# tberriel/OVO

Measured on AMD Instinct MI355X. Metric: frames/s (CLIP+SAM2+fusion+query), 640x480 ScanNet, 1/2/4/8 MI355X, higher is better.
Workload: dtype bf16; 1 GPU; BASELINE.json configs[2]: PE-Core-L14-336 TextRegion descriptors (2 x 336^2 crops of a 640x480 frame) + SAM2 hiera_b+ image encoder @1024^2 + back-projection + cull/project/match/vote on a 1000000-point map + multi-view fusion + dense per-point fusion + 10-prompt instance and dense-map query; every frame a keyframe; masks from the precomputed-mask seam (32/frame); map_points=1000000, texts=10, masks_per_frame=32, sam2=image encoder, masks=precomputed-mask seam (mask_generator.py:94-95), encoder_batch=14, dense_query=resident class map, rows touched by the keyframe re-evaluated, parallelism=single GPU, points_end=1366868, instances_end=242

## Files before the change

### include/ovo_hip.h

```cpp
#ifndef OVO_HIP_H
#define OVO_HIP_H

#include <stddef.h>
#include <stdint.h>

#ifdef __cplusplus
extern "C" {
#endif

#define OVO_OK 0
#define OVO_E_ARG (-1)
#define OVO_E_LAUNCH (-2)
#define OVO_E_UNSUPPORTED (-3)

typedef void *ovo_stream_t;

const char *ovo_hip_last_error(void);
int ovo_hip_abi_version(void);

int ovo_marker(int id, ovo_stream_t stream);
int ovo_profile_start(void);
int ovo_profile_stop(double *ms, double *work, int64_t *launches, int n_kinds);
int ovo_profile_bytes(double *bytes, int n_kinds);

// ... 80 lines not shown


typedef struct {
    const void *A; int64_t lda;
    const void *W; int64_t ldw;
    const float *bias;
    void *C; int64_t ldc;
    const float *add; int64_t ld_add;
    int32_t M, N, K;
    int32_t in_dtype, out_dtype, act;
    float alpha;
} ovo_gemm_t;
int ovo_gemm(const ovo_gemm_t *g, ovo_stream_t stream);
typedef struct {
    const float *cos, *sin;
    int32_t T, hd, cols, t0;
} ovo_rope_t;
int ovo_gemm_rope(const ovo_gemm_t *g, const ovo_rope_t *rope, ovo_stream_t stream);
int ovo_gemm_periodic(const ovo_gemm_t *g, int64_t add_rows, ovo_stream_t stream);
typedef struct {
    int32_t B, H, W, wh, ww;
} ovo_window_t;
int ovo_gemm_unwindow(const ovo_gemm_t *g, const ovo_window_t *win, ovo_stream_t stream);
int ovo_gemm_rowln(const ovo_gemm_t *g, const ovo_window_t *win, const float *ln_g, const float *ln_b, float eps, void *ln_out, int64_t ld_ln,
                   ovo_stream_t stream);
int ovo_gemm_fold_out(const ovo_gemm_t *g, void *xb, int64_t ld_xb, float *stats, int64_t ld_stats, ovo_stream_t stream);
int ovo_gemm_fold_stats(const float *x, int64_t ldx, int M, int D, void *xb, int64_t ld_xb, float *stats, ovo_stream_t stream);
int ovo_gemm_fold_in(const ovo_gemm_t *g, const ovo_rope_t *rope, const float *stats, int64_t ld_stats, int parts, int D, const float *rowsum, float eps,
                     ovo_stream_t stream);
int ovo_gemm_f32a(const ovo_gemm_t *g, const ovo_window_t *win, const float *x, int d, const float *gamma, const float *beta,
                  float eps, int mode, int pool2x2, ovo_stream_t stream);
int ovo_mlp_f32(float *x, int64_t rows, int d, const float *ln_g, const float *ln_b, float eps, const void *w1, int64_t ldw1,
                const float *b1, int hidden, const void *w2, int64_t ldw2, const float *b2, ovo_stream_t stream);
int ovo_window_attention_f32(const float *x, int B, int H, int W, int window, int d, int d_out, int heads, int pool, const float *ln_g,
                             const float *ln_b, float eps, const void *qkv_w, int64_t ldw, const float *qkv_b, void *att, int ld_att,
                             ovo_stream_t stream);
int ovo_gemm_argmax(const ovo_gemm_t *g, uint64_t *best, int store_scores, int n_valid, ovo_stream_t stream);
int ovo_decode_best(const uint64_t *best, int64_t n, float th, int64_t *out_cls, float *out_conf, ovo_stream_t stream);

typedef struct {
    const void *q, *k, *v;
    void *o;
    int64_t q_sb, q_sh, q_st, k_sb, k_sh, k_st, v_sb, v_sh, v_st, o_sb, o_sh, o_st;
    int32_t B, H, Tq, Tk, hd;
    float scale;
    int32_t causal;
} ovo_attention_t;
int ovo_attention(const ovo_attention_t *a, ovo_stream_t stream);

int ovo_gemm_fewrows(const ovo_gemm_t *g, ovo_stream_t stream);
int ovo_attention_short(const void *qkv, int B, int T, int H, int hd, float scale, void *out, ovo_stream_t stream);
int ovo_merge_clips(const float *logits, int64_t ld_logits, int per_row, const float *clips, int B, int D, float *out, ovo_stream_t stream);

int ovo_layernorm(const float *x, int64_t x_stride, int64_t rows, int d, const float *gamma, const float *beta,
                  float eps, void *y, int64_t y_stride, int out_dtype, ovo_stream_t stream);

int ovo_vit_embed(const float *patch, const float *prefix, int n_prefix, const float *pos, int B, int P, int d,
                  const float *gamma, const float *beta, float eps, float *x, ovo_stream_t stream);

int ovo_im2col(const float *img, int B, int C, int H, int W, int ksz, int stride, int pad, void *out, int kpad,
               ovo_stream_t stream);

int ovo_resize_normalize(const void *src, int src_dtype, int C, int H, int W, int y0, int x0, int ch, int cw,
                         float *out, int oh, int ow, int antialias, float scale, const float *mean3_host,
                         const float *std3_host, ovo_stream_t stream);

// ... 225 lines not shown
```

### ovo_amd/_lib.py

```python
from __future__ import annotations

import ctypes as C
import os
from typing import Optional

import torch

_HERE = os.path.dirname(os.path.abspath(__file__))
SO_PATH = os.path.join(_HERE, "lib", "libovo_hip.so")
ABI_VERSION = 15
E_UNSUPPORTED = -3


class OvoHipError(RuntimeError):
    pass


class Camera(C.Structure):
    _fields_ = [("aabb", C.c_float * 6), ("planes", C.c_float * 24), ("w2c", C.c_float * 16),
                ("K", C.c_float * 9), ("th", C.c_float), ("h", C.c_int32), ("w", C.c_int32)]


class Ratio(C.Structure):
    _fields_ = [("enabled", C.c_int32), ("r_h", C.c_float), ("r_w", C.c_float), ("crop_edge", C.c_int32)]


_P, _I64, _I32, _F32, _SZ = C.c_void_p, C.c_int64, C.c_int, C.c_float, C.c_size_t
_CAM = C.POINTER(Camera)


class Gemm(C.Structure):
    _fields_ = [("A", _P), ("lda", _I64), ("W", _P), ("ldw", _I64), ("bias", _P), ("C", _P), ("ldc", _I64),
                ("add", _P), ("ld_add", _I64), ("M", C.c_int32), ("N", C.c_int32), ("K", C.c_int32),
                ("in_dtype", C.c_int32), ("out_dtype", C.c_int32), ("act", C.c_int32), ("alpha", _F32)]


class Rope(C.Structure):
    _fields_ = [("cos", _P), ("sin", _P), ("T", C.c_int32), ("hd", C.c_int32), ("cols", C.c_int32), ("t0", C.c_int32)]


class Window(C.Structure):
    _fields_ = [(n, C.c_int32) for n in ("B", "H", "W", "wh", "ww")]

# ... 109 lines not shown
    "ovo_mask_or": (_I32, [_P, _I64, _P, _I32, _P]),
    "ovo_gather_rows": (_I32, [_P, _I64, _P, _I32, _P, _P]),
    "ovo_mask_area": (_I32, [_P, _I64, _P, _I32, _P, _P]),
    "ovo_gemm": (_I32, [C.POINTER(Gemm), _P]),
    "ovo_gemm_argmax": (_I32, [C.POINTER(Gemm), _P, _I32, _I32, _P]),
    "ovo_gemm_rope": (_I32, [C.POINTER(Gemm), C.POINTER(Rope), _P]),
    "ovo_gemm_periodic": (_I32, [C.POINTER(Gemm), _I64, _P]),
    "ovo_gemm_unwindow": (_I32, [C.POINTER(Gemm), C.POINTER(Window), _P]),
    "ovo_gemm_fold_out": (_I32, [C.POINTER(Gemm), _P, _I64, _P, _I64, _P]),
    "ovo_gemm_fold_stats": (_I32, [_P, _I64, _I32, _I32, _P, _I64, _P, _P]),
    "ovo_gemm_fold_in": (_I32, [C.POINTER(Gemm), C.POINTER(Rope), _P, _I64, _I32, _I32, _P, _F32, _P]),
    "ovo_gemm_rowln": (_I32, [C.POINTER(Gemm), C.POINTER(Window), _P, _P, _F32, _P, _I64, _P]),
    "ovo_gemm_f32a": (_I32, [C.POINTER(Gemm), C.POINTER(Window), _P, C.c_int, _P, _P, C.c_float, C.c_int, C.c_int, _P]),
    "ovo_decode_best": (_I32, [_P, _I64, _F32, _P, _P, _P]),
    "ovo_attention": (_I32, [C.POINTER(Attention), _P]),
    "ovo_gemm_fewrows": (_I32, [C.POINTER(Gemm), _P]),
    "ovo_attention_short": (_I32, [_P, _I32, _I32, _I32, _I32, _F32, _P, _P]),
    "ovo_merge_clips": (_I32, [_P, _I64, _I32, _P, _I32, _I32, _P, _P]),
    "ovo_layernorm": (_I32, [_P, _I64, _I64, _I32, _P, _P, _F32, _P, _I64, _I32, _P]),
    "ovo_vit_embed": (_I32, [_P, _P, _I32, _P, _I32, _I32, _I32, _P, _P, _F32, _P, _P]),
    "ovo_im2col": (_I32, [_P, _I32, _I32, _I32, _I32, _I32, _I32, _I32, _P, _I32, _P]),
    "ovo_resize_normalize": (_I32, [_P, _I32, _I32, _I32, _I32, _I32, _I32, _I32, _I32, _P, _I32, _I32, _I32, _F32,
                                    C.POINTER(C.c_float), C.POINTER(C.c_float), _P]),
    "ovo_resize_normalize_batch": (_I32, [_P, _I32, _I32, _I32, _I32, _I32, _P, _I32, _P, _I32, _I32, _I32, _F32, _P, _P, _P]),
    "ovo_resize_window_normalize": (_I32, [_P, _I32, _I32, _I32, _I32, _I32, _I32, _I32, _I32, _P, _I32, _I32, _I32, _I32, _I32, _I32, _I32, _F32,
                                           C.POINTER(C.c_float), C.POINTER(C.c_float), _P]),
    "ovo_rope_qk": (_I32, [_P, _I32, _I32, _I32, _I32, _P, _P, _I32, _P]),
    "ovo_feature_masks": (_I32, [_P, _I32, _I32, _I32, _I32, _I32, _P, _I32, _P, _P]),
    "ovo_stitch_tokens_t": (_I32, [_P, _I32, _I32, _I32, _I32, _I32, _I32, _P, _I32, _P]),
    "ovo_unit_tokens": (_I32, [_P, _I32, _I32, _I32, _P, _P, _P]),
    "ovo_global_patch_filter": (_I32, [_P, _P, _I32, _I32, _I32, _F32, _P, _P]),
    "ovo_scale_rows_bf16": (_I32, [_P, _P, _I32, _I32, _P, _P]),
    "ovo_mlp_f32": (_I32, [_P, _I64, _I32, _P, _P, _F32, _P, _I64, _P, _I32, _P, _I64, _P, _P]),
    "ovo_window_attention_f32": (_I32, [_P, _I32, _I32, _I32, _I32, _I32, _I32, _I32, _I32, _P, _P, _F32, _P, _I64, _P, _P, _I32, _P]),
    "ovo_l2_normalize_rows": (_I32, [_P, _I64, _I32, _P, _P]),
    "ovo_cast_f32": (_I32, [_P, _I64, _P, _I32, _P]),
    "ovo_row_epilogue": (_I32, [_P, _I64, _I32, _P, _I64, _P, _P, _F32, _P, _I64, _P, _P, _P, _P]),
    "ovo_sam_upscale_ln": (_I32, [_P, _P, _P, _P, _P, _F32, _I64, _I32, _I32, _P, _P]),
    "ovo_sam_upscale_masks": (_I32, [_P, _P, _P, _P, _I32, _I32, _I64, _I32, _I32, _P, _P]),
    "ovo_sam_linear": (_I32, [_P, _P, _P, _P, _I64, _I32, _P, _I32, _I64, _I32, _I32, _P]),
    "ovo_sam_proj_ln": (_I32, [_P, _P, _P, _P, _P, _I64, _P, _P, _F32, _P, _I64, _P, _P, _P, _I64, _I32, _I32, _P]),
    "ovo_sam_up1_ln": (_I32, [_P, _P, _P, _P, _P, _P, _F32, _I64, _I32, _I32, _I32, _P, _P]),
    "ovo_sam_up2_masks": (_I32, [_P, _P, _P, _P, _P, _I32, _I32, _I64, _I32, _I32, _I32, _P, _P]),
    "ovo_instance_moments": (_I32, [_P, _P, _I64, _I32, _P, _P, _P]),
    "ovo_near_fraction": (_I32, [_P, _P, _P, _I32, _I64, _F32, _P, _P]),
    "ovo_remap_instances": (_I32, [_P, _I64, _P, _I32, _P]),
    "ovo_map_reanchor_workspace_bytes": (_SZ, [_I32]),
    "ovo_map_reanchor": (_I32, [_P, _P, _P, _P, _I64, _P, _P, _P, _P, _I64, _P, _P, _P, _I32, _P, _SZ, _P]),
    "ovo_sam_i2t_attention": (_I32, [_P, _I64, _I32, _P, _P, _P, _I64, _I32, _I32, _I32, _F32, _P]),
    "ovo_sam_t2i_attention": (_I32, [_P, _P, _P, _I64, _I32, _P, _I64, _I32, _I32, _I32, _F32, _P]),
    "ovo_paint_segmap": (_I32, [_P, _I32, _I64, _P, _P]),
    "ovo_amg_mask_stats": (_I32, [_P, _I32, _I32, _I32, _I32, _I32, _F32, _F32, _P, _P]),
    "ovo_amg_binarize": (_I32, [_P, _P, _I32, _I32, _I32, _I32, _I32, _F32, _P, _P]),
    "ovo_vit_workspace_bytes": (_SZ, [C.POINTER(VitConfig), _I32]),
    "ovo_vit_forward": (_I32, [C.POINTER(VitConfig), C.POINTER(VitWeights), _P, _I32, _P, _P, _SZ, _P]),
    "ovo_hiera_workspace_bytes": (_SZ, [C.POINTER(HieraConfig), _I32]),
    "ovo_hiera_forward": (_I32, [C.POINTER(HieraConfig), C.POINTER(HieraWeights), _P, _I32, _P, _P, _P, _P, _SZ, _P]),
    "ovo_hiera_patch_embed": (_I32, [_P, _I32, _I32, _I32, _P, _I32, _P, _P, _P, _P]),
    "ovo_eval_cell_keys": (_I32, [_P, _I64, C.POINTER(EvalGrid), _P, _P]),
    "ovo_eval_grid_records": (_I32, [_P, _P, _I64, _P, _P]),
    "ovo_knn5_labels": (_I32, [_P, _P, _I64, C.POINTER(EvalGrid), _P, _P, _I64, _P, _P, _P, _P, _P, _P]),
    "ovo_confusion": (_I32, [_P, _P, _I64, _I32, C.POINTER(C.c_int64), _I32, _P, _P, _P]),
}

_lib: Optional[C.CDLL] = None

# ... 173 lines not shown
```

### ovo_amd/build.py

```python
from __future__ import annotations

import concurrent.futures as cf
import os
import shutil
import subprocess
import sys

HERE = os.path.dirname(os.path.abspath(__file__))
CSRC = os.path.join(HERE, "csrc")
OUT_DIR = os.path.join(HERE, "lib")
OBJ_DIR = os.path.join(OUT_DIR, "obj")
SO = os.path.join(OUT_DIR, "libovo_hip.so")
ARCH = "gfx950"

COMMON = ["--offload-arch=" + ARCH, "-O3", "-std=c++17", "-fPIC", "-Wall", "-Wno-unused-function",
          "-Wno-unused-result", "-I" + os.path.join(os.path.dirname(HERE), "include")]
EXTRA = {"geometry.hip": ["-ffp-contract=off"], "evalknn.hip": ["-ffp-contract=off"], "mlp_stream.hip": ["-fno-slp-vectorize"], "gemm_stream.hip": ["-fno-slp-vectorize"],
         "winattn.hip": ["-fno-slp-vectorize"], "gemm8p.hip": ["-fno-slp-vectorize"],
         "merger.hip": ["-fno-slp-vectorize"]}


def hipcc() -> str:
    for c in (os.environ.get("HIPCC"), shutil.which("hipcc"), "/opt/rocm/bin/hipcc"):
        if c and os.path.exists(c):
            return c
    raise RuntimeError("hipcc not found: libovo_hip.so cannot be built")


def sources():
    return sorted(f for f in os.listdir(CSRC) if f.endswith(".hip"))


def _stale(target: str, deps) -> bool:
    if not os.path.exists(target):
        return True
    t = os.path.getmtime(target)
    return any(os.path.getmtime(d) > t for d in deps)


def _run(cmd, what: str) -> None:
    r = subprocess.run(cmd, capture_output=True, text=True)
    if r.returncode != 0:
        raise RuntimeError(f"{what} failed:\n{r.stdout}\n{r.stderr}")
    if r.stderr.strip():
        sys.stderr.write(r.stderr)


def _compile(src: str, flags, force: bool) -> bool:
    obj = os.path.join(OBJ_DIR, src.replace(".hip", ".o"))
    deps = [os.path.join(CSRC, src)] + [os.path.join(CSRC, h) for h in os.listdir(CSRC) if h.endswith(".h")]
    deps.append(os.path.join(os.path.dirname(HERE), "include", "ovo_hip.h"))
# ... 36 lines not shown
```

### ovo_amd/csrc/core.hip

```cpp
#include <stdarg.h>
#include <stdio.h>
#include <stdlib.h>

#include <string.h>

#include <atomic>
#include <chrono>
#include <vector>

#include "common.h"

static thread_local char g_err[512] = "";

void ovo_set_error(const char *fmt, ...) {
    va_list ap;
    va_start(ap, fmt);
    vsnprintf(g_err, sizeof(g_err), fmt, ap);
    va_end(ap);
}

namespace {
struct Rec { hipEvent_t a, b; int kind; double work, bytes; int shape[3], flags; int cslot; double per_item, fixed; };
struct Prof {
    bool on = false;
// ... 40 lines not shown
    if (!g_prof.on || g_prof.recs.empty() || !device_count) return;
    if (!g_prof.counts && hipHostMalloc((void **)&g_prof.counts, SLOTS * sizeof(int32_t), hipHostMallocDefault) != hipSuccess) { g_prof.counts = nullptr; return; }
    if (g_prof.n_counts >= SLOTS) return;
    Rec &r = g_prof.recs.back();
    r.cslot = g_prof.n_counts++; r.per_item = per_item; r.fixed = fixed;
    (void)hipMemcpyAsync(g_prof.counts + r.cslot, device_count, sizeof(int32_t), hipMemcpyDeviceToHost, s);
}

template <typename T>
static int host_wait(const T *flag, T value, int64_t timeout_us) {
    OVO_REQUIRE(flag, "null flag");
    const volatile T *f = flag;
    const auto t0 = std::chrono::steady_clock::now();
    for (unsigned spin = 0;; ++spin) {
        if (*f == value) { std::atomic_thread_fence(std::memory_order_acquire); return OVO_OK; }
        if ((spin & 255) == 255 &&
            std::chrono::duration_cast<std::chrono::microseconds>(std::chrono::steady_clock::now() - t0).count() > timeout_us) {
            ovo_set_error("ovo_host_wait: timed out after %lld us (flag %lld, expected %lld)", (long long)timeout_us, (long long)*f, (long long)value);
            return OVO_E_LAUNCH;
        }
        __builtin_ia32_pause();
    }
}

__global__ void k_marker(int id, int *sink) { if (sink && id < 0) *sink = id; }

extern "C" {
int ovo_marker(int id, ovo_stream_t stream) {
    k_marker<<<1, 1, 0, (hipStream_t)stream>>>(id, nullptr);
    OVO_CHECK_LAUNCH();
    return OVO_OK;
}
const char *ovo_hip_last_error(void) { return g_err; }
int ovo_hip_abi_version(void) { return 15; }

int ovo_profile_start(void) {
    g_prof.recs.clear();
    g_prof.used = 0;
    g_prof.n_counts = 0;
    g_prof.on = true;
    return OVO_OK;
}

int ovo_profile_stop(double *ms, double *work, int64_t *launches, int n_kinds) {
    g_prof.on = false;
    OVO_REQUIRE(ms && work && launches && n_kinds > 0 && n_kinds <= OVO_PROF_KINDS, "bad argument");
    for (int i = 0; i < n_kinds; ++i) { ms[i] = 0; work[i] = 0; launches[i] = 0; }
    for (int i = 0; i < OVO_PROF_KINDS; ++i) g_last_bytes[i] = 0;
    OVO_HIP(hipDeviceSynchronize());
    FILE *dump = getenv("OVO_PROF_DUMP") ? fopen(getenv("OVO_PROF_DUMP"), "a") : nullptr;
    for (const Rec &r : g_prof.recs) {
        float t = 0.f;
        if (hipEventElapsedTime(&t, r.a, r.b) != hipSuccess || r.kind >= n_kinds) continue;
        double wk = r.work, by = r.bytes;
        if (r.cslot >= 0 && g_prof.counts) wk = by = r.per_item * (double)g_prof.counts[r.cslot] + r.fixed;
        ms[r.kind] += t; work[r.kind] += wk; launches[r.kind] += 1; g_last_bytes[r.kind] += by;
        if (dump) fprintf(dump, "%d %d %d %d %.0f %.4f %d\n", r.kind, r.shape[0], r.shape[1], r.shape[2], wk, t, r.flags);
    }
    if (dump) fclose(dump);
    g_prof.recs.clear();
    g_prof.used = 0;
    return OVO_OK;
}

int ovo_profile_bytes(double *bytes, int n_kinds) {
    OVO_REQUIRE(bytes && n_kinds > 0 && n_kinds <= OVO_PROF_KINDS, "bad argument");
    for (int i = 0; i < n_kinds; ++i) bytes[i] = g_last_bytes[i];
// ... 18 lines not shown
```

### ovo_amd/csrc/gemm_common.h

```cpp
#pragma once
#include <hip/hip_bf16.h>
#include <hip/hip_fp16.h>

#include "common.h"

namespace ovo_gemm_detail {

typedef __attribute__((ext_vector_type(8))) __bf16 bf16x8;
typedef __attribute__((ext_vector_type(8))) _Float16 f16x8;
typedef __attribute__((ext_vector_type(4))) float f32x4;

struct GemmArgs {
    const char *A; long long lda;
    const char *W; long long ldw;
    const float *bias;
    void *C; long long ldc;
    const float *add; long long ld_add;
    int M, N, K;
    int out_dtype, act;
    float alpha;
    int nbn;
    int chunk, tiles;
    int add_rows;
    int strip;
// ... 205 lines not shown
}

inline double gemm_algorithmic_bytes(const GemmArgs &g) {
    const double mn = (double)g.M * g.N, a_bytes = g.ln_mode ? (double)g.M * g.ln_d * 4.0 : (double)g.M * g.K * 2.0;
    return a_bytes + (double)g.N * g.K * 2.0 + mn * (g.out_dtype == 0 ? 4.0 : 2.0) + (g.add ? (g.add_rows > 0 ? (double)g.add_rows * g.N * 4.0 : mn * 4.0) : 0.0) +
           (g.bias ? g.N * 4.0 : 0.0) +
           (g.xb_out ? mn * 2.0 + (double)g.M * (g.N / 64) * 8.0 : 0.0) +
           (g.fold_stats ? (double)g.M * g.fold_parts * 8.0 + g.N * 4.0 : 0.0);
}

inline bool knob_gemm_no_chunk() { return ovo_knob_set("OVO_GEMM_NO_CHUNK"); }
inline bool knob_gemm_no_stream() { return ovo_knob_set("OVO_GEMM_NO_STREAM"); }
inline OvoKnobStr knob_gemm_tile() { return ovo_knob_str("OVO_GEMM_TILE"); }
inline bool knob_gelu_poly() { return ovo_knob_set("OVO_GELU_POLY"); }
inline bool knob_8p_no_slab16() { return ovo_knob_set("OVO_8P_NO_SLAB16"); }

int gemm8p_launch(const GemmArgs &g, int bn, int in_dtype, hipStream_t s);

struct FoldOut { void *xb; long long ld_xb; float *stats; long long ld_stats; };
struct FoldIn { const float *stats; long long ld_stats; int parts; int D; const float *colsum; float eps; };
int gemm_fold_parts(int N);
bool gemm_fold_ok(int M, int N, int K);
int gemm_fold_producer(const ovo_gemm_t *p, const FoldOut &o, ovo_stream_t stream);
int gemm_fold_consumer(const ovo_gemm_t *p, const ovo_rope_t *rope, const FoldIn &f, ovo_stream_t stream);
int gemm_fold_rowstats(const float *x, long long ldx, int M, int D, void *xb, long long ld_xb, float *stats, ovo_stream_t stream);
int gemm8q_launch(const GemmArgs &g, int in_dtype, hipStream_t s);
int gemm_stream_launch(const GemmArgs &g, int in_dtype, hipStream_t s);
int gemm_f32a_stream(const ovo_gemm_t *p, const ovo_window_t *win, const float *x, int d, const float *gamma, const float *beta, float eps, int mode,
                     int pool2x2, ovo_stream_t stream, uint16_t *qpool_out = nullptr, int qpool_cols = 0);

int mlp_stream_launch(float *x, long long rows, int d, const float *ln_g, const float *ln_b, float eps, const void *w1, long long ldw1, const float *b1,
                      int hid, const void *w2, long long ldw2, const float *b2, hipStream_t s);

int gemm_unwindow_rowln(const ovo_gemm_t *p, const ovo_window_t *win, const float *ln_g, const float *ln_b, float eps, void *ln_out, long long ld_ln,
                        ovo_stream_t stream);

int win_attn_launch(const float *x, int B, int H, int W, int ws, int d, int d_out, int heads, int pool, const float *ln_g, const float *ln_b, float eps,
                    const void *qkv_w, long long ldw, const float *qkv_b, void *att, int ld_att, hipStream_t s);

}
```

### ovo_amd/csrc/hiera.hip

```cpp
#include "gemm_common.h"

namespace {

__device__ __forceinline__ uint16_t f2bf(float x) {
    const __bf16 h = (__bf16)x;
    return *(const uint16_t *)&h;
}
__device__ __forceinline__ float bf2f(uint16_t v) { return __uint_as_float((uint32_t)v << 16); }

struct Grid {
    int B, H, W, ws;
    int nwh, nww, wh, ww;
    long long rows;
};
__host__ __device__ inline Grid make_grid(int B, int H, int W, int ws) {
    Grid g; g.B = B; g.H = H; g.W = W; g.ws = ws;
    if (ws > 0) { g.wh = g.ww = ws; g.nwh = (H + ws - 1) / ws; g.nww = (W + ws - 1) / ws; }
    else { g.wh = H; g.ww = W; g.nwh = g.nww = 1; }
    g.rows = (long long)B * g.nwh * g.nww * g.wh * g.ww;
    return g;
}
__device__ __forceinline__ long long row_of(const Grid &g, int b, int y, int x) {
    const int wy = y / g.wh, wx = x / g.ww;
    return ((((long long)b * g.nwh + wy) * g.nww + wx) * g.wh + (y - wy * g.wh)) * g.ww + (x - wx * g.ww);
// ... 136 lines not shown
        float m = -3.0e38f;
#pragma unroll
        for (int dy = 0; dy < 2; ++dy)
#pragma unroll
            for (int dx = 0; dx < 2; ++dx) m = fmaxf(m, rows[row_of(g, b, 2 * y + dy, 2 * x + dx) * C + c]);
        out[i] = m;
    }
}

__global__ void __launch_bounds__(256) k_cast_pad(const float *__restrict__ x, long long rows, int C, int kp, uint16_t *__restrict__ y) {
    if (C % 4 == 0 && kp % 4 == 0) {
        const int k4 = kp >> 2;
        const long long total = rows * k4;
        for (long long i = (long long)blockIdx.x * blockDim.x + threadIdx.x; i < total; i += (long long)gridDim.x * blockDim.x) {
            const int c = (int)(i % k4) * 4;
            const long long r = i / k4;
            uint2 p = make_uint2(0u, 0u);
            if (c < C) {
                const float4 v = *(const float4 *)(x + r * C + c);
                p.x = f2bf(v.x) | ((uint32_t)f2bf(v.y) << 16);
                p.y = f2bf(v.z) | ((uint32_t)f2bf(v.w) << 16);
            }
            *(uint2 *)(y + r * kp + c) = p;
        }
        return;
    }
    const long long total = rows * kp;
    for (long long i = (long long)blockIdx.x * blockDim.x + threadIdx.x; i < total; i += (long long)gridDim.x * blockDim.x) {
        const int c = (int)(i % kp);
        y[i] = c < C ? f2bf(x[(i / kp) * C + c]) : (uint16_t)0;
    }
}

__global__ void __launch_bounds__(256) k_topdown_add(float *__restrict__ fine, const float *__restrict__ coarse, int B, int H, int W, int C) {
    const int c4 = C >> 2;
    const long long total = (long long)B * H * W * c4;
    for (long long i = (long long)blockIdx.x * blockDim.x + threadIdx.x; i < total; i += (long long)gridDim.x * blockDim.x) {
        const int c = (int)(i % c4);
        long long t = i / c4;
        const int x = (int)(t % W); t /= W;
        const int y = (int)(t % H);
        const int b = (int)(t / H);
        const float4 u = ((const float4 *)coarse)[(((long long)b * (H / 2) + y / 2) * (W / 2) + x / 2) * c4 + c];
        float4 v = ((float4 *)fine)[i];
        v.x += u.x; v.y += u.y; v.z += u.z; v.w += u.w;
        ((float4 *)fine)[i] = v;
    }
}

inline int padk(int v) { return (v + 63) / 64 * 64; }
inline size_t align256(size_t v) { return (v + 255) & ~(size_t)255; }

struct Plan {
    int n_blocks;
    int dim_in[64], dim_out[64], heads[64], ws[64], pool[64], Hin[64];
    int stage_end[64];
};

int make_plan(const ovo_hiera_config_t &c, Plan &p) {
    int idx = 0, H = c.image_size / 4;
    for (int s = 0; s < 4; ++s)
        for (int b = 0; b < c.blocks[s]; ++b) {
            if (idx >= 64) return -1;
            const bool first = s > 0 && b == 0;
            p.dim_in[idx] = first ? c.dims[s - 1] : c.dims[s];
            p.dim_out[idx] = c.dims[s];
            p.heads[idx] = c.heads[s];
            int ws = first ? c.window[s - 1] : c.window[s];
            for (int k = 0; k < c.n_global; ++k) if (c.global_blocks[k] == idx) ws = 0;
            p.ws[idx] = ws;
            p.pool[idx] = first;
            p.Hin[idx] = H;
            if (first) H /= 2;
            p.stage_end[idx] = b == c.blocks[s] - 1 ? s : -1;
            ++idx;
        }
    p.n_blocks = idx;
    return 0;
}

struct Ws {
    uint16_t *col; float *x, *xr, *tmp; uint16_t *h, *qkv, *qp, *att, *u, *cast; float *lat[4];
    size_t bytes;
};

Ws carve(const ovo_hiera_config_t &c, const Plan &p, int B, void *base) {
    size_t max_x = 0, max_h = 0, max_qkv = 0, max_att = 0, max_u = 0, max_tmp = 0, max_cast = 0;
    for (int i = 0; i < p.n_blocks; ++i) {
        const int H = p.Hin[i], Ho = p.pool[i] ? H / 2 : H;
        const Grid g = make_grid(B, H, H, p.ws[i]);
        const size_t tok_in = (size_t)B * H * H, tok_out = (size_t)B * Ho * Ho;
        const size_t rows_out = p.pool[i] ? (size_t)g.rows / 4 : (size_t)g.rows;
        max_x = max_x > tok_in * p.dim_in[i] ? max_x : tok_in * p.dim_in[i];
        max_x = max_x > tok_out * p.dim_out[i] ? max_x : tok_out * p.dim_out[i];
        size_t v = (size_t)g.rows * padk(p.dim_in[i]); max_h = max_h > v ? max_h : v;
        v = tok_out * padk(p.dim_out[i]); max_h = max_h > v ? max_h : v;
        v = (size_t)g.rows * 3 * p.dim_out[i]; max_qkv = max_qkv > v ? max_qkv : v;
        v = rows_out * padk(p.dim_out[i]); max_att = max_att > v ? max_att : v;
        v = tok_out * 4 * p.dim_out[i]; max_u = max_u > v ? max_u : v;
        v = (size_t)g.rows * p.dim_out[i]; max_tmp = max_tmp > v ? max_tmp : v;
        v = tok_out * padk(p.dim_out[i]); max_cast = max_cast > v ? max_cast : v;
    }
    const size_t T0 = (size_t)B * (c.image_size / 4) * (c.image_size / 4);
    max_cast = max_cast > T0 * c.fpn_dim ? max_cast : T0 * c.fpn_dim;
    Ws w;
    char *b0 = (char *)base;
    size_t off = 0;
    auto take = [&](size_t n) { char *r = b0 ? b0 + off : nullptr; off += align256(n); return r; };
    w.col = (uint16_t *)take(T0 * 192 * 2);
    w.x = (float *)take(max_x * 4);
    w.xr = (float *)take(max_x * 4);
    w.tmp = (float *)take(max_tmp * 4);
    w.h = (uint16_t *)take(max_h * 2);
    w.qkv = (uint16_t *)take(max_qkv * 2);
    w.qp = (uint16_t *)take(max_att * 2);
    w.att = (uint16_t *)take(max_att * 2);
    w.u = (uint16_t *)take(max_u * 2);
    w.cast = (uint16_t *)take(max_cast * 2);
    for (int s = 0; s < 4; ++s) { const size_t t = T0 >> (2 * s); w.lat[s] = (float *)take(t * c.fpn_dim * 4); }
    w.bytes = off;
    return w;
}

int gemm(const void *A, long long lda, const void *W, long long ldw, const float *bias, void *C, long long ldc, int out_dtype,
         const float *add, long long ld_add, long long M, int N, int K, int act, ovo_stream_t s) {
    ovo_gemm_t g;
    g.A = A; g.lda = lda; g.W = W; g.ldw = ldw; g.bias = bias; g.C = C; g.ldc = ldc; g.add = add; g.ld_add = ld_add;
    g.M = (int)M; g.N = N; g.K = K; g.in_dtype = 2; g.out_dtype = out_dtype; g.act = act; g.alpha = 1.0f;
    return ovo_gemm(&g, s);
}

int gemm_from_f32(const float *x, const Grid &g, int d, int kp, const float *gamma, const float *beta, float eps, int mode, uint16_t *h, bool &h_done,
                  const void *W, const float *bias, void *C, long long ldc, int out_dtype, int N, int act, ovo_stream_t s) {
    ovo_gemm_t q;
    q.A = h; q.lda = kp; q.W = W; q.ldw = kp; q.bias = bias; q.C = C; q.ldc = ldc; q.add = nullptr; q.ld_add = 0;
    q.M = (int)g.rows; q.N = N; q.K = kp; q.in_dtype = 2; q.out_dtype = out_dtype; q.act = act; q.alpha = 1.0f;
    if (!h_done) {
        const ovo_window_t w = {g.B, g.H, g.W, g.wh, g.ww};
        const int rc = ovo_gemm_detail::gemm_f32a_stream(&q, g.ws > 0 ? &w : nullptr, x, d, gamma, beta, eps, mode, 0, s);
        if (rc != OVO_E_UNSUPPORTED) return rc;
        OVO_REQUIRE(d <= 2048 && g.rows < (1ll << 31), "LayerNorm rows of more than 2048 columns / more than 2^31 rows");
        if (mode == 1) launch_ln_window(x, g, d, kp, gamma, beta, eps, h, (hipStream_t)s);
        else k_cast_pad<<<ovo_grid(g.rows * kp, 256), 256, 0, (hipStream_t)s>>>(x, g.rows, d, kp, h);
        h_done = true;
    }
    return ovo_gemm(&q, s);
}

constexpr int PE_TH = 8, PE_TW = 32, PE_IH = 4 * PE_TH + 3, PE_RS = 136, PE_WS = 200;
template <int NT>
__global__ void __launch_bounds__(512) __attribute__((amdgpu_waves_per_eu(4, 4))) k_patch_embed7(const float *__restrict__ img, int S, const uint16_t *__restrict__ w, int ldw,
                                                      const float *__restrict__ bias, const float *__restrict__ pos, float *__restrict__ out, int B,
// ... 276 lines not shown
            og.A = k.att; og.lda = kout; og.W = L.out_w; og.ldw = kout; og.bias = L.out_b; og.C = x; og.ldc = dout; og.add = residual; og.ld_add = dout;
            og.M = (int)(n_win * tq); og.N = dout; og.K = kout; og.in_dtype = 2; og.out_dtype = 0; og.act = 0; og.alpha = 1.0f;
            const ovo_window_t ow = {go.B, go.H, go.W, go.wh, go.ww};
            const bool rowln = ovo_knob_set("OVO_HIERA_PROJ_LN");
            int rc = OVO_E_UNSUPPORTED;
            if (rowln && dout == 448 && kout == dout)
                rc = ovo_gemm_detail::gemm_unwindow_rowln(&og, &ow, L.ln2_g, L.ln2_b, c.ln_eps, k.h, kout, stream);
            if (rc == OVO_OK) ln2_done = true;
            else if (rc != OVO_E_UNSUPPORTED) return rc;
            else TRY(ovo_gemm_unwindow(&og, &ow, stream));
        }
        const Grid gi = make_grid(B, Ho, Ho, 0);
        h_done = false;
        const long long chunk_mb = ovo_knob_int("OVO_HIERA_MLP_CHUNK_MB", 0);
        const long long hid_row = (long long)4 * dout * 2;
        long long chunk_rows = chunk_mb > 0 ? (chunk_mb << 20) / hid_row / 4096 * 4096 : 0;
        if (chunk_rows <= 0 || tok_out < 2 * chunk_rows || tok_out * hid_row <= (200ll << 20)) chunk_rows = tok_out;
        const int fused = ovo_gemm_detail::mlp_stream_launch(x, tok_out, dout, L.ln2_g, L.ln2_b, c.ln_eps, L.fc1_w, kout, L.fc1_b, 4 * dout, L.fc2_w, 4 * dout, L.fc2_b, hs);
        if (fused != OVO_OK && fused != OVO_E_UNSUPPORTED) return fused;
        for (long long r0 = fused == OVO_OK ? tok_out : 0; r0 < tok_out; r0 += chunk_rows) {
            const long long nr = tok_out - r0 < chunk_rows ? tok_out - r0 : chunk_rows;
            const Grid gc = chunk_rows == tok_out ? gi : make_grid(1, (int)nr, 1, 0);
            bool h_ready = chunk_rows == tok_out ? (h_done || ln2_done) : false;
            float *xc = x + r0 * dout;
            TRY(gemm_from_f32(xc, gc, dout, kout, L.ln2_g, L.ln2_b, c.ln_eps, 1, k.h, h_ready, L.fc1_w, L.fc1_b, k.u, 4 * dout, 2, 4 * dout, 1, stream));
            TRY(gemm(k.u, 4 * dout, L.fc2_w, 4 * dout, L.fc2_b, xc, dout, 0, xc, dout, nr, dout, 4 * dout, 0, stream));
        }
        h_done = false;
        LAUNCHED();

        if (p.stage_end[i] >= 0) {
            const int s = p.stage_end[i];
            OVO_REQUIRE(w->neck_w[s] && w->neck_b[s], "missing neck weights");
            bool cast_done = false;
            TRY(gemm_from_f32(x, gi, dout, kout, nullptr, nullptr, 0.f, 2, k.cast, cast_done, w->neck_w[s], w->neck_b[s], k.lat[s], c.fpn_dim, 0,
                              c.fpn_dim, 0, stream));
        }
    }
    const int S16 = c.image_size / 16;
    k_topdown_add<<<ovo_grid((long long)B * S16 * S16 * (c.fpn_dim / 4), 256), 256, 0, hs>>>(k.lat[2], k.lat[3], B, S16, S16, c.fpn_dim);
    LAUNCHED();
    OVO_HIP(hipMemcpyAsync(feat2, k.lat[2], (size_t)B * S16 * S16 * c.fpn_dim * 4, hipMemcpyDeviceToDevice, hs));
    const long long t0 = (long long)B * T0, t1 = t0 / 4;
    if (c.hi_res) {
        OVO_REQUIRE(w->s0_w && w->s0_b && w->s1_w && w->s1_b, "missing conv_s0 / conv_s1 weights");
        bool cast_done = false;
        const Grid g0 = make_grid(B, S4, S4, 0), g1 = make_grid(B, S4 / 2, S4 / 2, 0);
        TRY(gemm_from_f32(k.lat[0], g0, c.fpn_dim, c.fpn_dim, nullptr, nullptr, 0.f, 2, k.cast, cast_done, w->s0_w, w->s0_b, feat0, 32, 0, 32, 0, stream));
        cast_done = false;
        TRY(gemm_from_f32(k.lat[1], g1, c.fpn_dim, c.fpn_dim, nullptr, nullptr, 0.f, 2, k.cast, cast_done, w->s1_w, w->s1_b, feat1, 64, 0, 64, 0, stream));
    } else {
        OVO_HIP(hipMemcpyAsync(feat0, k.lat[0], (size_t)t0 * c.fpn_dim * 4, hipMemcpyDeviceToDevice, hs));
        OVO_HIP(hipMemcpyAsync(feat1, k.lat[1], (size_t)t1 * c.fpn_dim * 4, hipMemcpyDeviceToDevice, hs));
    }
    LAUNCHED();
    return OVO_OK;
}

}
```

Measured before the change: 473.9 frames/s.

## Fuse Hiera neck lateral projection with conv_s0/s1 into one streaming kernel

For the two high-resolution stages, the neck 1x1 projection to fpn_dim and the following conv_s0/conv_s1 projection are fused into a single MFMA kernel. The kernel keeps the 256-wide intermediate in registers and double-buffers weight chunks into LDS via buffer-to-LDS loads. This avoids writing the large fp32 lateral maps for stages 0 and 1, recasting them to bf16 and re-reading them. The top-down add also writes straight into feat2 when it is aligned, dropping a device-to-device copy. The trade-off is a specialised kernel with hard-coded shapes, and the intermediate is rounded to bf16 before the second product.

```diff
diff --git a/include/ovo_hip.h b/include/ovo_hip.h
--- a/include/ovo_hip.h
+++ b/include/ovo_hip.h
@@ -136,6 +136,8 @@
                   float eps, int mode, int pool2x2, ovo_stream_t stream);
 int ovo_mlp_f32(float *x, int64_t rows, int d, const float *ln_g, const float *ln_b, float eps, const void *w1, int64_t ldw1,
                 const float *b1, int hidden, const void *w2, int64_t ldw2, const float *b2, ovo_stream_t stream);
+int ovo_neck_f32(const float *x, int64_t rows, int d, const void *w1, int64_t ldw1, const float *b1, int hidden, const void *w2, int64_t ldw2,
+                 const float *b2, float *out, int n_out, ovo_stream_t stream);
 int ovo_window_attention_f32(const float *x, int B, int H, int W, int window, int d, int d_out, int heads, int pool, const float *ln_g,
                              const float *ln_b, float eps, const void *qkv_w, int64_t ldw, const float *qkv_b, void *att, int ld_att,
                              ovo_stream_t stream);
diff --git a/ovo_amd/_lib.py b/ovo_amd/_lib.py
--- a/ovo_amd/_lib.py
+++ b/ovo_amd/_lib.py
@@ -8,7 +8,7 @@
 
 _HERE = os.path.dirname(os.path.abspath(__file__))
 SO_PATH = os.path.join(_HERE, "lib", "libovo_hip.so")
-ABI_VERSION = 15
+ABI_VERSION = 16
 E_UNSUPPORTED = -3
 
 
@@ -184,6 +184,7 @@
     "ovo_global_patch_filter": (_I32, [_P, _P, _I32, _I32, _I32, _F32, _P, _P]),
     "ovo_scale_rows_bf16": (_I32, [_P, _P, _I32, _I32, _P, _P]),
     "ovo_mlp_f32": (_I32, [_P, _I64, _I32, _P, _P, _F32, _P, _I64, _P, _I32, _P, _I64, _P, _P]),
+    "ovo_neck_f32": (_I32, [_P, _I64, _I32, _P, _I64, _P, _I32, _P, _I64, _P, _P, _I32, _P]),
     "ovo_window_attention_f32": (_I32, [_P, _I32, _I32, _I32, _I32, _I32, _I32, _I32, _I32, _P, _P, _F32, _P, _I64, _P, _P, _I32, _P]),
     "ovo_l2_normalize_rows": (_I32, [_P, _I64, _I32, _P, _P]),
     "ovo_cast_f32": (_I32, [_P, _I64, _P, _I32, _P]),
diff --git a/ovo_amd/build.py b/ovo_amd/build.py
--- a/ovo_amd/build.py
+++ b/ovo_amd/build.py
@@ -17,6 +17,7 @@
           "-Wno-unused-result", "-I" + os.path.join(os.path.dirname(HERE), "include")]
 EXTRA = {"geometry.hip": ["-ffp-contract=off"], "evalknn.hip": ["-ffp-contract=off"], "mlp_stream.hip": ["-fno-slp-vectorize"], "gemm_stream.hip": ["-fno-slp-vectorize"],
          "winattn.hip": ["-fno-slp-vectorize"], "gemm8p.hip": ["-fno-slp-vectorize"],
+         "neck_stream.hip": ["-fno-slp-vectorize"],
          "merger.hip": ["-fno-slp-vectorize"]}
 
 
diff --git a/ovo_amd/csrc/core.hip b/ovo_amd/csrc/core.hip
--- a/ovo_amd/csrc/core.hip
+++ b/ovo_amd/csrc/core.hip
@@ -96,7 +96,7 @@
     return OVO_OK;
 }
 const char *ovo_hip_last_error(void) { return g_err; }
-int ovo_hip_abi_version(void) { return 15; }
+int ovo_hip_abi_version(void) { return 16; }
 
 int ovo_profile_start(void) {
     g_prof.recs.clear();
diff --git a/ovo_amd/csrc/gemm_common.h b/ovo_amd/csrc/gemm_common.h
--- a/ovo_amd/csrc/gemm_common.h
+++ b/ovo_amd/csrc/gemm_common.h
@@ -261,6 +261,10 @@
 int mlp_stream_launch(float *x, long long rows, int d, const float *ln_g, const float *ln_b, float eps, const void *w1, long long ldw1, const float *b1,
                       int hid, const void *w2, long long ldw2, const float *b2, hipStream_t s);
 
+bool neck_stream_covers(long long rows, int d, long long ldw1, int hid, int n_out);
+int neck_stream_launch(const float *x, long long rows, int d, const void *w1, long long ldw1, const float *b1, int hid, const void *w2, long long ldw2,
+                       const float *b2, float *out, int n_out, hipStream_t s);
+
 int gemm_unwindow_rowln(const ovo_gemm_t *p, const ovo_window_t *win, const float *ln_g, const float *ln_b, float eps, void *ln_out, long long ld_ln,
                         ovo_stream_t stream);
 
diff --git a/ovo_amd/csrc/hiera.hip b/ovo_amd/csrc/hiera.hip
--- a/ovo_amd/csrc/hiera.hip
+++ b/ovo_amd/csrc/hiera.hip
@@ -192,7 +192,7 @@
     }
 }
 
-__global__ void __launch_bounds__(256) k_topdown_add(float *__restrict__ fine, const float *__restrict__ coarse, int B, int H, int W, int C) {
+__global__ void __launch_bounds__(256) k_topdown_add(const float *__restrict__ fine, const float *__restrict__ coarse, float *__restrict__ out, int B, int H, int W, int C) {
     const int c4 = C >> 2;
     const long long total = (long long)B * H * W * c4;
     for (long long i = (long long)blockIdx.x * blockDim.x + threadIdx.x; i < total; i += (long long)gridDim.x * blockDim.x) {
@@ -202,9 +202,9 @@
         const int y = (int)(t % H);
         const int b = (int)(t / H);
         const float4 u = ((const float4 *)coarse)[(((long long)b * (H / 2) + y / 2) * (W / 2) + x / 2) * c4 + c];
-        float4 v = ((float4 *)fine)[i];
+        float4 v = ((const float4 *)fine)[i];
         v.x += u.x; v.y += u.y; v.z += u.z; v.w += u.w;
-        ((float4 *)fine)[i] = v;
+        ((float4 *)out)[i] = v;
     }
 }
 
@@ -244,6 +244,12 @@
     size_t bytes;
 };
 
+bool neck_fused(const ovo_hiera_config_t &c, int B, int s) {
+    if (!c.hi_res || s > 1 || ovo_knob_set("OVO_HIERA_NECK_TWO_PASS")) return false;
+    const long long rows = ((long long)B * (c.image_size / 4) * (c.image_size / 4)) >> (2 * s);
+    return ovo_gemm_detail::neck_stream_covers(rows, c.dims[s], padk(c.dims[s]), c.fpn_dim, s == 0 ? 32 : 64);
+}
+
 Ws carve(const ovo_hiera_config_t &c, const Plan &p, int B, void *base) {
     size_t max_x = 0, max_h = 0, max_qkv = 0, max_att = 0, max_u = 0, max_tmp = 0, max_cast = 0;
     for (int i = 0; i < p.n_blocks; ++i) {
@@ -277,7 +283,7 @@
     w.att = (uint16_t *)take(max_att * 2);
     w.u = (uint16_t *)take(max_u * 2);
     w.cast = (uint16_t *)take(max_cast * 2);
-    for (int s = 0; s < 4; ++s) { const size_t t = T0 >> (2 * s); w.lat[s] = (float *)take(t * c.fpn_dim * 4); }
+    for (int s = 0; s < 4; ++s) { const size_t t = T0 >> (2 * s); w.lat[s] = neck_fused(c, B, s) ? nullptr : (float *)take(t * c.fpn_dim * 4); }
     w.bytes = off;
     return w;
 }
@@ -620,23 +626,36 @@
         if (p.stage_end[i] >= 0) {
             const int s = p.stage_end[i];
             OVO_REQUIRE(w->neck_w[s] && w->neck_b[s], "missing neck weights");
+            if (neck_fused(c, B, s)) {
+                const void *cw = s == 0 ? w->s0_w : w->s1_w;
+                const float *cb = s == 0 ? w->s0_b : w->s1_b;
+                float *feat = s == 0 ? feat0 : feat1;
+                OVO_REQUIRE(cw && cb, "missing conv_s0 / conv_s1 weights");
+                OVO_REQUIRE((((uintptr_t)feat | (uintptr_t)w->neck_w[s] | (uintptr_t)cw) & 15) == 0, "feat0 / feat1 and the neck weights must be 16-byte aligned");
+                TRY(ovo_gemm_detail::neck_stream_launch(x, tok_out, dout, w->neck_w[s], kout, w->neck_b[s], c.fpn_dim, cw, c.fpn_dim, cb, feat, s == 0 ? 32 : 64, hs));
+                LAUNCHED();
+                continue;
+            }
             bool cast_done = false;
             TRY(gemm_from_f32(x, gi, dout, kout, nullptr, nullptr, 0.f, 2, k.cast, cast_done, w->neck_w[s], w->neck_b[s], k.lat[s], c.fpn_dim, 0,
                               c.fpn_dim, 0, stream));
         }
     }
     const int S16 = c.image_size / 16;
-    k_topdown_add<<<ovo_grid((long long)B * S16 * S16 * (c.fpn_dim / 4), 256), 256, 0, hs>>>(k.lat[2], k.lat[3], B, S16, S16, c.fpn_dim);
+    float *top = ((uintptr_t)feat2 & 15) == 0 ? feat2 : k.lat[2];
+    k_topdown_add<<<ovo_grid((long long)B * S16 * S16 * (c.fpn_dim / 4), 256), 256, 0, hs>>>(k.lat[2], k.lat[3], top, B, S16, S16, c.fpn_dim);
     LAUNCHED();
-    OVO_HIP(hipMemcpyAsync(feat2, k.lat[2], (size_t)B * S16 * S16 * c.fpn_dim * 4, hipMemcpyDeviceToDevice, hs));
+    if (top != feat2) OVO_HIP(hipMemcpyAsync(feat2, top, (size_t)B * S16 * S16 * c.fpn_dim * 4, hipMemcpyDeviceToDevice, hs));
     const long long t0 = (long long)B * T0, t1 = t0 / 4;
     if (c.hi_res) {
         OVO_REQUIRE(w->s0_w && w->s0_b && w->s1_w && w->s1_b, "missing conv_s0 / conv_s1 weights");
         bool cast_done = false;
         const Grid g0 = make_grid(B, S4, S4, 0), g1 = make_grid(B, S4 / 2, S4 / 2, 0);
-        TRY(gemm_from_f32(k.lat[0], g0, c.fpn_dim, c.fpn_dim, nullptr, nullptr, 0.f, 2, k.cast, cast_done, w->s0_w, w->s0_b, feat0, 32, 0, 32, 0, stream));
+        if (!neck_fused(c, B, 0))
+            TRY(gemm_from_f32(k.lat[0], g0, c.fpn_dim, c.fpn_dim, nullptr, nullptr, 0.f, 2, k.cast, cast_done, w->s0_w, w->s0_b, feat0, 32, 0, 32, 0, stream));
         cast_done = false;
-        TRY(gemm_from_f32(k.lat[1], g1, c.fpn_dim, c.fpn_dim, nullptr, nullptr, 0.f, 2, k.cast, cast_done, w->s1_w, w->s1_b, feat1, 64, 0, 64, 0, stream));
+        if (!neck_fused(c, B, 1))
+            TRY(gemm_from_f32(k.lat[1], g1, c.fpn_dim, c.fpn_dim, nullptr, nullptr, 0.f, 2, k.cast, cast_done, w->s1_w, w->s1_b, feat1, 64, 0, 64, 0, stream));
     } else {
         OVO_HIP(hipMemcpyAsync(feat0, k.lat[0], (size_t)t0 * c.fpn_dim * 4, hipMemcpyDeviceToDevice, hs));
         OVO_HIP(hipMemcpyAsync(feat1, k.lat[1], (size_t)t1 * c.fpn_dim * 4, hipMemcpyDeviceToDevice, hs));
diff --git a/ovo_amd/csrc/neck_stream.hip b/ovo_amd/csrc/neck_stream.hip
--- /dev/null
+++ b/ovo_amd/csrc/neck_stream.hip
@@ -0,0 +1,235 @@
+#include <type_traits>
+
+#include "skinny.h"
+
+using namespace ovo_gemm_detail;
+
+namespace {
+
+struct NeckArgs {
+    const float *x; long long rows;
+    const uint16_t *w1; long long ldw1; const float *b1;
+    const uint16_t *w2; long long ldw2; const float *b2;
+    float *out;
+};
+
+template <int K1, int D, int HID, int NOUT, int RB, int NTHREADS, int HC>
+__global__ void __launch_bounds__(NTHREADS) k_neck_stream(NeckArgs g, int n_slots) {
+#if __HIP_DEVICE_COMPILE__
+    constexpr int NCH = HID / HC, KS1 = K1 / 32, KS2 = HC / 32, NT2 = NOUT / 16;
+    constexpr int CPR1 = K1 / 8, CPR2 = HC / 8;
+    constexpr int W1_BYTES = HC * K1 * 2, W2_BYTES = NOUT * HC * 2, BUF = W1_BYTES + W2_BYTES;
+    constexpr int P1 = HC * CPR1, P2 = NOUT * CPR2, PIECES = P1 + P2, PPT = (PIECES + NTHREADS - 1) / NTHREADS;
+    constexpr int WPB = NTHREADS / 64;
+    static_assert(HID % HC == 0 && HC % 32 == 0 && NOUT % 16 == 0 && K1 % 32 == 0 && K1 >= D && D % 8 == 0, "shape");
+    static_assert(P1 % 64 == 0 && P2 % 64 == 0, "a wave instruction must not straddle the two blocks");
+    using S1 = ovo_skinny::Skinny<K1, HC>;
+    using S2 = ovo_skinny::Skinny<HC, NOUT>;
+    extern __shared__ __attribute__((aligned(16))) char smem[];
+    __shared__ __attribute__((aligned(16))) float b1s[HID];
+    __shared__ __attribute__((aligned(16))) float b2s[NOUT];
+    const int tid = threadIdx.x, lane = tid & 63, wave = tid >> 6, fr = lane & 15, fq = lane >> 4;
+
+    auto unit_of = [](int q) { const int j = q >> 4, n = q & 15; return 32 * (j >> 1) + 8 * (n >> 2) + 4 * (j & 1) + (n & 3); };
+    for (int i = tid; i < HID; i += NTHREADS) b1s[i] = g.b1[(i / HC) * HC + unit_of(i % HC)];
+    for (int i = tid; i < NOUT; i += NTHREADS) b2s[i] = g.b2[i];
+
+    auto piece_off = [&](int id) -> long long {
+        if (id < P1) { const int q = id / CPR1, c = (id % CPR1) ^ S1::swz(q); return unit_of(q) * g.ldw1 + c * 8; }
+        const int n = (id - P1) / CPR2, c = ((id - P1) % CPR2) ^ S2::swz(n);
+        return n * g.ldw2 + c * 8;
+    };
+
+    bf16x8 af[RB][KS1];
+    long long row[RB];
+    auto load_rows = [&](long long grp) {
+        const long long blocks = (g.rows + 15) / 16;
+#pragma unroll
+        for (int rb = 0; rb < RB; ++rb) {
+            const long long b = (grp * WPB + wave) * RB + rb;
+            const long long m = b * 16 + fr;
+            row[rb] = (b < blocks && m < g.rows) ? m : -1;
+            const float *xp = g.x + (row[rb] < 0 ? 0 : row[rb]) * D;
+#pragma unroll
+            for (int ks = 0; ks < KS1; ++ks) {
+                const int d0 = (ks * 4 + fq) * 8;
+                float4 lo = make_float4(0.f, 0.f, 0.f, 0.f), hi = lo;
+                if (row[rb] >= 0 && d0 < D) { lo = *(const float4 *)(xp + d0); hi = *(const float4 *)(xp + d0 + 4); }
+                uint32_t pk[4] = {pack_bf16(lo.x, lo.y), pack_bf16(lo.z, lo.w), pack_bf16(hi.x, hi.y), pack_bf16(hi.z, hi.w)};
+                af[rb][ks] = *(const bf16x8 *)pk;
+            }
+        }
+    };
+    f32x4 acc2[RB][NT2];
+    auto products = [&](const char *w1, const char *w2, int c) {
+        const float *bc = b1s + c * HC + fq * 4;
+#pragma unroll
+        for (int kp = 0; kp < KS2; ++kp) {
+            f32x4 acc1[RB][2];
+#pragma unroll
+            for (int rb = 0; rb < RB; ++rb) acc1[rb][0] = acc1[rb][1] = f32x4{0.f, 0.f, 0.f, 0.f};
+#pragma unroll
+            for (int ks = 0; ks < KS1; ++ks) {
+                const char *wp = w1 + (fr * CPR1 + ((ks * 4 + fq) ^ S1::swz(fr))) * 16 + (2 * kp) * (16 * CPR1 * 16);
+                const bf16x8 wa = *(const bf16x8 *)wp, wb = *(const bf16x8 *)(wp + 16 * CPR1 * 16);
+#pragma unroll
+                for (int rb = 0; rb < RB; ++rb) {
+                    acc1[rb][0] = Mfma<bf16x8>::run(wa, af[rb][ks], acc1[rb][0]);
+                    acc1[rb][1] = Mfma<bf16x8>::run(wb, af[rb][ks], acc1[rb][1]);
+                }
+            }
+            bf16x8 hf[RB];
+#pragma unroll
+            for (int rb = 0; rb < RB; ++rb) {
+                uint32_t pk[4];
+#pragma unroll
+                for (int h = 0; h < 2; ++h) {
+                    const f32x4 bv = *(const f32x4 *)(bc + (2 * kp + h) * 16);
+                    pk[2 * h] = pack_bf16(acc1[rb][h][0] + bv[0], acc1[rb][h][1] + bv[1]);
+                    pk[2 * h + 1] = pack_bf16(acc1[rb][h][2] + bv[2], acc1[rb][h][3] + bv[3]);
+                }
+                hf[rb] = *(const bf16x8 *)pk;
+            }
+            bf16x8 w[NT2];
+            const char *wp = w2 + (fr * CPR2 + ((kp * 4 + fq) ^ S2::swz(fr))) * 16;
+#pragma unroll
+            for (int j = 0; j < NT2; ++j) w[j] = *(const bf16x8 *)(wp + j * (16 * CPR2 * 16));
+#pragma unroll
+            for (int j = 0; j < NT2; ++j)
+#pragma unroll
+                for (int rb = 0; rb < RB; ++rb) acc2[rb][j] = Mfma<bf16x8>::run(w[j], hf[rb], acc2[rb][j]);
+            __builtin_amdgcn_sched_barrier(0);
+        }
+    };
+    auto store_rows = [&]() {
+#pragma unroll
+        for (int rb = 0; rb < RB; ++rb) {
+            if (row[rb] < 0) continue;
+            float *op = g.out + row[rb] * NOUT + fq * 4;
+            const float *bc = b2s + fq * 4;
+#pragma unroll
+            for (int j = 0; j < NT2; ++j) {
+                const f32x4 bv = *(const f32x4 *)(bc + j * 16);
+                *(float4 *)(op + j * 16) = make_float4(acc2[rb][j][0] + bv[0], acc2[rb][j][1] + bv[1], acc2[rb][j][2] + bv[2], acc2[rb][j][3] + bv[3]);
+            }
+        }
+    };
+    auto zero_acc2 = [&]() {
+#pragma unroll
+        for (int rb = 0; rb < RB; ++rb)
+#pragma unroll
+            for (int j = 0; j < NT2; ++j) acc2[rb][j] = f32x4{0.f, 0.f, 0.f, 0.f};
+    };
+
+    const long long blocks = (g.rows + 15) / 16, groups = (blocks + WPB * RB - 1) / (WPB * RB);
+    if constexpr (NCH == 1) {
+        for (int id = tid; id < PIECES; id += NTHREADS)
+            *(uint4 *)(smem + id * 16) = *(const uint4 *)((id < P1 ? g.w1 : g.w2) + piece_off(id));
+        __syncthreads();
+        for (long long grp = blockIdx.x; grp < groups; grp += n_slots) {
+            load_rows(grp);
+            zero_acc2();
+            products(smem, smem + W1_BYTES, 0);
+            store_rows();
+        }
+    } else {
+        int src_off[PPT];
+#pragma unroll
+        for (int p = 0; p < PPT; ++p) {
+            const int id = p * NTHREADS + tid;
+            src_off[p] = id < PIECES ? (int)piece_off(id) : 0;
+        }
+        const __amdgpu_buffer_rsrc_t rs1 = __builtin_amdgcn_make_buffer_rsrc((void *)g.w1, 0, (int)((long long)HID * g.ldw1 * 2), 0x00020000);
+        const __amdgpu_buffer_rsrc_t rs2 = __builtin_amdgcn_make_buffer_rsrc((void *)g.w2, 0, (int)((long long)NOUT * g.ldw2 * 2), 0x00020000);
+        auto dma = [&](int chunk, auto BUF_) {
+            char *base = smem + decltype(BUF_)::value * BUF;
+#pragma unroll
+            for (int p = 0; p < PPT; ++p) {
+                const int id0 = p * NTHREADS + wave * 64;
+                if (id0 >= PIECES) continue;
+                if (id0 < P1) __builtin_amdgcn_raw_ptr_buffer_load_lds(rs1, (__attribute__((address_space(3))) void *)(base + id0 * 16), 16, src_off[p] * 2, chunk * HC * (int)g.ldw1 * 2, 0, 0);
+                else __builtin_amdgcn_raw_ptr_buffer_load_lds(rs2, (__attribute__((address_space(3))) void *)(base + id0 * 16), 16, src_off[p] * 2, chunk * HC * 2, 0, 0);
+            }
+        };
+        auto chunk_body = [&](auto PAR_, int c) {
+            constexpr int PAR = decltype(PAR_)::value;
+            asm volatile("s_waitcnt vmcnt(0)" ::: "memory");
+            __builtin_amdgcn_sched_barrier(0);
+            __syncthreads();
+            __builtin_amdgcn_sched_barrier(0);
+            if (c + 1 < NCH) dma(c + 1, std::integral_constant<int, PAR ^ 1>{});
+            __builtin_amdgcn_sched_barrier(0);
+            products(smem + PAR * BUF, smem + PAR * BUF + W1_BYTES, c);
+        };
+        for (long long grp = blockIdx.x; grp < groups; grp += n_slots) {
+            __syncthreads();
+            dma(0, std::integral_constant<int, 0>{});
+            load_rows(grp);
+            zero_acc2();
+            int c = 0;
+            for (; c + 1 < NCH; c += 2) {
+                chunk_body(std::integral_constant<int, 0>{}, c);
+                chunk_body(std::integral_constant<int, 1>{}, c + 1);
+            }
+            if (c < NCH) chunk_body(std::integral_constant<int, 0>{}, c);
+            store_rows();
+        }
+    }
+#endif
+}
+
+template <int K1, int D, int HID, int NOUT, int RB, int NTHREADS, int HC>
+int launch_neck(const NeckArgs &g, hipStream_t s) {
+    constexpr size_t lds = (size_t)(HID == HC ? 1 : 2) * (HC * K1 * 2 + NOUT * HC * 2);
+    constexpr size_t lds_all = lds + (size_t)(HID + NOUT) * sizeof(float) + 64;
+    static_assert(lds_all <= 160 * 1024, "LDS");
+    constexpr int BY_LDS = (int)((160 * 1024) / (lds_all + 1024)), BY_WAVES = NTHREADS >= 512 ? 1 : 512 / NTHREADS;
+    constexpr int PER_CU = BY_LDS < BY_WAVES ? BY_LDS : BY_WAVES;
+    constexpr size_t lds_launch = (PER_CU == 1 && lds_all < 82 * 1024) ? lds + (82 * 1024 - lds_all) : lds;
+    static bool attr_done = false;
+    if (!attr_done) {
+        hipError_t e = hipFuncSetAttribute((const void *)k_neck_stream<K1, D, HID, NOUT, RB, NTHREADS, HC>, hipFuncAttributeMaxDynamicSharedMemorySize, (int)lds_launch);
+        if (e != hipSuccess) { ovo_set_error("ovo_neck_f32: hipFuncSetAttribute: %s", hipGetErrorString(e)); return OVO_E_LAUNCH; }
+        attr_done = true;
+    }
+    const long long blocks = (g.rows + 15) / 16, groups = (blocks + (NTHREADS / 64) * RB - 1) / ((NTHREADS / 64) * RB);
+    const int slots = (int)(groups < 256 * PER_CU ? groups : 256 * PER_CU);
+    const bool prof = ovo_prof_enabled();
+    if (prof) { ovo_prof_begin(8, 2.0 * (double)g.rows * HID * (double)(K1 + NOUT), s); ovo_prof_shape((int)g.rows, NOUT, K1); ovo_prof_flags(1 | 64);
+                ovo_prof_bytes(4.0 * (double)g.rows * (D + NOUT) + 2.0 * HID * (K1 + NOUT) + 4.0 * (HID + NOUT)); }
+    k_neck_stream<K1, D, HID, NOUT, RB, NTHREADS, HC><<<slots, NTHREADS, lds_launch, s>>>(g, slots);
+    if (prof) ovo_prof_end(s);
+    return OVO_OK;
+}
+
+}
+
+namespace ovo_gemm_detail {
+
+bool neck_stream_covers(long long rows, int d, long long ldw1, int hid, int n_out) {
+    if (knob_gemm_no_stream() || knob_gemm_tile().set) return false;
+    return rows >= 16384 && rows < (1ll << 31) && hid == 256 && ((d == 112 && ldw1 == 128 && n_out == 32) || (d == 224 && ldw1 == 256 && n_out == 64));
+}
+
+int neck_stream_launch(const float *x, long long rows, int d, const void *w1, long long ldw1, const float *b1, int hid, const void *w2, long long ldw2,
+                       const float *b2, float *out, int n_out, hipStream_t s) {
+    if (!neck_stream_covers(rows, d, ldw1, hid, n_out) || !x || !w1 || !b1 || !w2 || !b2 || !out) return OVO_E_UNSUPPORTED;
+    if (ldw2 < hid || ldw2 % 8 != 0 || (((uintptr_t)w1 | (uintptr_t)w2 | (uintptr_t)x | (uintptr_t)out) & 15) != 0) return OVO_E_UNSUPPORTED;
+    NeckArgs g;
+    g.x = x; g.rows = rows; g.w1 = (const uint16_t *)w1; g.ldw1 = ldw1; g.b1 = b1; g.w2 = (const uint16_t *)w2; g.ldw2 = ldw2; g.b2 = b2; g.out = out;
+    if (d == 112) return launch_neck<128, 112, 256, 32, 2, 1024, 256>(g, s);
+    if (d == 224) return launch_neck<256, 224, 256, 64, 2, 512, 64>(g, s);
+    return OVO_E_UNSUPPORTED;
+}
+
+}
+
+extern "C" int ovo_neck_f32(const float *x, int64_t rows, int d, const void *w1, int64_t ldw1, const float *b1, int hidden, const void *w2, int64_t ldw2,
+                            const float *b2, float *out, int n_out, ovo_stream_t stream) {
+    OVO_REQUIRE(x && w1 && b1 && w2 && b2 && out && rows >= 0 && d > 0 && hidden > 0 && n_out > 0, "bad argument");
+    if (rows == 0) return OVO_OK;
+    const int rc = ovo_gemm_detail::neck_stream_launch(x, rows, d, w1, ldw1, b1, hidden, w2, ldw2, b2, out, n_out, (hipStream_t)stream);
+    if (rc != OVO_OK) return rc;
+    OVO_CHECK_LAUNCH();
+    return OVO_OK;
+}
```

Measured after the change: 480.6 frames/s, median of 6. 1.4% higher.
